# djamahl99/findnpropagate

Measured on AMD Instinct MI355X. Metric: NuScenes scenes/s (30k pts, Transfusion voxel backbone), higher is better.
Workload: dtype bf16

## Files before the change

### findnpropagate_amd/backbones_3d/spconv_backbone.py

```python
from functools import partial

import os
import torch
import torch.nn as nn

from .. import sparse as S
from .. import spconv


def replace_feature(out, new_features):
    return out.replace_feature(new_features)


def post_act_block(in_channels, out_channels, kernel_size, indice_key=None, stride=1, padding=0,
                   conv_type='subm', norm_fn=None):
    if conv_type == 'subm':
        conv = spconv.SubMConv3d(in_channels, out_channels, kernel_size, bias=False, indice_key=indice_key)
    elif conv_type == 'spconv':
        conv = spconv.SparseConv3d(in_channels, out_channels, kernel_size, stride=stride, padding=padding,
                                   bias=False, indice_key=indice_key)
    elif conv_type == 'inverseconv':
        conv = spconv.SparseInverseConv3d(in_channels, out_channels, kernel_size, indice_key=indice_key, bias=False)
    else:
        raise NotImplementedError
# ... 266 lines not shown


TWO_STREAMS = {"0": False, "1": True}.get(os.environ.get("FNP_TWO_STREAMS", ""))


class _PointsGraph:
    FAR = 1.0e9

    def __init__(self, engine, capacity, n_feat, batch_size, voxel_cfg, device, probe=False, split_index=False):
        self.probe, self.deferred = bool(probe), []
        self.host_counts = not self.probe
        self.split_index, self.graph_i, self._index_cut = bool(split_index), None, False
        self.counts_dev = None
        if self.host_counts:
            self.counts_pin = torch.zeros((32,), dtype=torch.int32, pin_memory=True)
            self._pin_np = self.counts_pin.numpy()
            self.counts_seq, self._replays = torch.zeros((1,), dtype=torch.int32, device=device), 0
        else:
            self.counts_pin = torch.empty((16,), dtype=torch.int32, pin_memory=True)
            self.graph_b, self.counts_event = torch.cuda.CUDAGraph(), torch.cuda.Event()
        self.done_event = torch.cuda.Event()
        self._replayed = False
        self.engine, self.capacity, self.batch_size = engine, capacity, batch_size
        self.pts = torch.full((capacity, n_feat), self.FAR, dtype=torch.float32, device=device)
        self.off = torch.zeros((batch_size + 1,), dtype=torch.int32, device=device)
        self.n_prev = 0
        self.prep_key = engine._prep_key
        engine._gate_hold = True
        try:
            self._body(voxel_cfg)
        finally:
            engine._gate_hold = False
        torch.cuda.synchronize(device)
        self.cap_factor = engine._graph_key()
        self.graph = torch.cuda.CUDAGraph()
        import gc
        gc_was_on = gc.isenabled()
        gc.collect()
        gc.disable()
        try:
            if self.split_index:
                self.graph_i = torch.cuda.CUDAGraph()
                self._ctx = torch.cuda.graph(self.graph_i)
            else:
                self._ctx = torch.cuda.graph(self.graph)
            self._ctx.__enter__()
            try:
                self.vox, self.res = self._body(voxel_cfg, capture=True)
            finally:
                self._ctx.__exit__(None, None, None)
            assert self.counts_dev is not None and (self.deferred or not self.probe), "the engine did not reach its cut"
            assert self._index_cut or not self.split_index, "the engine did not cut behind its index chain"
        finally:
            if gc_was_on:
                gc.enable()

    def stage(self, points, batch_offsets):
        n = int(points.shape[0])
        if (points.is_cuda and points.dtype == torch.float32 and points.is_contiguous() and batch_offsets.is_cuda
                and batch_offsets.dtype == torch.int32 and batch_offsets.is_contiguous()):
            S.stage_points(points, batch_offsets, self.pts, self.off, self.n_prev, self.FAR)
        else:
            self.pts[:n].copy_(points, non_blocking=True)
            if self.n_prev > n:
                self.pts[n:self.n_prev].fill_(self.FAR)
            self.off.copy_(batch_offsets, non_blocking=True)
        self.n_prev = n

    def index_ready(self):
        if not self.split_index or self._index_cut:
            return
        self._index_cut = True
        self._ctx.__exit__(None, None, None)
        self._ctx = torch.cuda.graph(self.graph, pool=self.graph_i.pool())
        self._ctx.__enter__()

    def counts_ready(self, counts_dev):
        self.counts_dev = counts_dev
        if self.host_counts:
            return
        self._ctx.__exit__(None, None, None)
        self._ctx = torch.cuda.graph(self.graph_b, pool=(self.graph_i if self.split_index else self.graph).pool())
        self._ctx.__enter__()

    def replay(self, profile=None, conv_stream=None):
        cur = torch.cuda.current_stream(self.pts.device)
        if self._replayed:
            cur.wait_event(self.done_event)
        if self.engine._last_done is not None and self.engine._last_done is not self.done_event:
            cur.wait_event(self.engine._last_done)
# ... 33 lines not shown
        if self.host_counts:
            import time
            want, word, t0 = self._replays & 0xffffffff, self._pin_np, None
            spins = 0
            while (int(word[16]) & 0xffffffff) != want:
                spins += 1
                if spins > 3000:
                    time.sleep(5.0e-5)
                    if spins & 0x3f == 0:
                        t0 = t0 or time.monotonic()
                        if self.done_event.query() and (int(word[16]) & 0xffffffff) != want:
                            raise RuntimeError("the forward ended without its counts launch (sequence %d, expected %d)" % (int(word[16]), want))
                        if time.monotonic() - t0 > 60.0:
                            raise RuntimeError("no counts from the device after 60 s")
            return [int(v) for v in word[:self.counts_dev.numel()]]
        self.counts_event.synchronize()
        return self.counts_pin[:self.counts_dev.numel()].tolist()

    def _body(self, voxel_cfg, capture=False):
        e = self.engine
        e._ensure_clean()
        e._dirty = True
        grids = e._get_grids(self.batch_size, self.pts.device)
        vox = S.voxelize(self.pts, self.off, self.batch_size, voxel_cfg, grid=grids[0], workspace=e._vox_ws)
        e._vox_ws = vox['workspace']
        res = e._run_once(vox['mean'], vox['coords'], vox['n'], self.batch_size, grids[0], sync=False, n_cells=vox['n_cells'],
                          probe=self if capture else None)
        return vox, res


concurrent_streams = S.concurrent_streams


class PointsPipeline:

    def __init__(self, module, batch_size, voxel_cfg, depth=2, capacity=65536, n_feat=5, device=None, probe=False, serial_convs=None, streams=None):
        assert depth >= 1
        self.probe, self.profile = bool(probe), None
        self.module, self.batch_size, self.cfg, self.depth = module, int(batch_size), voxel_cfg, int(depth)
        self.capacity, self.n_feat = int(capacity), int(n_feat)
        self.device = device if device is not None else next(module.parameters()).device
        self.engines = [FusedResBackbone(module) for _ in range(self.depth)]
        for e in self.engines:
            e.two_streams = self.depth == 1

        self.serial_convs = self.depth > 1 and (bool(serial_convs) if serial_convs is not None else self.batch_size >= 8)
        if streams is not None:
# ... 590 lines not shown
```

### findnpropagate_amd/csrc/voxelize.hip

```cpp
#include "rankgrid.h"

namespace {

constexpr int kThreads = 256;
constexpr int kSentinel = 0x7f7f7f7f;
constexpr int kMaxBatch = 1024;

struct VoxWs {
    long long *code;
    int *rank;
    int *flag;
    int *top;
    int *cnt;
    int *scene;
    int *n_sorted;
    int *n_first;
    int *fscan;
    void *scan_ws;
};

__host__ long long align_up(long long v) { return (v + 255) & ~255ll; }

__host__ long long carve(VoxWs &w, char *base, long long n, int B, int cap, int maxp, long long nsum) {
    long long off = 0;
    auto take = [&](long long bytes) {
        char *p = base ? base + off : nullptr;
        off += align_up(bytes);
        return p;
    };
    w.code = (long long *)take(8 * n);
    w.rank = (int *)take(4 * n);
    w.flag = (int *)take(4 * n);
    w.fscan = (int *)take(4 * n);
    w.top = (int *)take(4ll * cap * maxp);
    w.cnt = (int *)take(4ll * cap + 4);
    w.scene = (int *)take(4ll * (3 * B + 8));
    w.n_sorted = (int *)take(4);
    w.n_first = (int *)take(4);
    const long long a = fnp_scan::rank_grid_workspace_bytes(nsum), b2 = fnp_scan::workspace_bytes(n);
    w.scan_ws = take(a > b2 ? a : b2);
    return off;
}

__device__ __forceinline__ int batch_of(const int *__restrict__ off, int B, int i) {
    int lo = 0, hi = B;
    while (hi - lo > 1) {
        const int mid = (lo + hi) >> 1;
        if (off[mid] <= i) lo = mid; else hi = mid;
    }
    return lo;
}

__global__ __launch_bounds__(kThreads) void vox_mark_kernel(const float *__restrict__ pts, int n, int C,
                                                            const int *__restrict__ boff, int B, fnp_voxel_cfg cfg,
                                                            RG g, long long *__restrict__ code, int *__restrict__ cnt) {
    {
        const int z = blockIdx.x * kThreads + threadIdx.x;
        if (z <= n) cnt[z] = 0;
        if (z == 0 && (long long)gridDim.x * kThreads <= n) cnt[n] = 0;
    }
    __shared__ MarkTab tab;
    mark_tab_init(&tab, threadIdx.x, kThreads);
    const int i = blockIdx.x * kThreads + threadIdx.x;
    const int lane = fnp_lane();
    long long blk = -1;
    unsigned long long m = 0ull;
    if (i < n) {
        const float *p = pts + (size_t)i * C;
        int c[3];
        bool ok = true;
#pragma unroll
        for (int j = 0; j < 3; ++j) {
            const float q = (p[j] - cfg.range_min[j]) / cfg.voxel_size[j];
            const float f = floorf(q);
            ok = ok && (f >= 0.f) && (f < (float)cfg.grid[j]);
            c[j] = (int)f;
        }
        long long cd = -1;
        if (ok) {
            const int i0 = __builtin_amdgcn_readfirstlane(i);
            int b = batch_of(boff, B, i0);
            if (b + 1 < B && i >= boff[b + 1]) b = batch_of(boff, B, i);
            blk = rg_block_of(g.d, b, c[2], c[1], c[0]);
            const int bit = rg_bit_of(c[2], c[1], c[0]);
            m = 1ull << bit;
            cd = (blk << 6) | bit;
        }
        code[i] = cd;
    }
#pragma unroll
    for (int d = 1; d < 64; d <<= 1) {
        const long long nb = __shfl_up(blk, d);
        const unsigned long long nm = __shfl_up(m, d);
        if (lane >= d && nb == blk) m |= nm;
    }
    const long long nxt = __shfl_down(blk, 1);
    if (blk >= 0 && (lane == 63 || nxt != blk)) mark_put(&tab, g, blk, m);
    mark_tab_flush(&tab, g, threadIdx.x, kThreads);
}

__global__ __launch_bounds__(kThreads) void vox_insert_kernel(int n, int maxp, int cap,
                                                              const unsigned long long *__restrict__ bits,
                                                              const unsigned *__restrict__ base,
                                                              const long long *__restrict__ code,
                                                              int *__restrict__ rank, int *__restrict__ top, int *__restrict__ cnt,
                                                              int *__restrict__ crowded, int *__restrict__ late) {
    const int i = blockIdx.x * kThreads + threadIdx.x;
    if (i >= n) return;
    late[i] = 0;
    const long long cd = code[i];
    int r = -1;
    if (cd >= 0) {
        const long long blk = cd >> 6;
        const int bit = (int)(cd & 63);
        r = (int)base[blk] + __popcll(bits[blk] & ((1ull << bit) - 1ull));
        if (r >= cap) r = -1;
    }
    rank[i] = r;
    if (r < 0) return;
    const int s = atomicAdd(&cnt[r], 1);
    if (s < maxp) {
// ... 12 lines not shown
    int carry = i;
    int *slots = top + (size_t)rank[i] * maxp;
    for (int j = 0; j < maxp; ++j) {
        const int old = atomicMin(&slots[j], carry);
        carry = old > carry ? old : carry;
    }
}

__global__ __launch_bounds__(kThreads) void vox_flag_kernel(int n, int maxp, const int *__restrict__ rank,
                                                            const int *__restrict__ top, const int *__restrict__ cnt, int *__restrict__ flag) {
    const int i = fnp_xcd_block() * kThreads + threadIdx.x;
    if (i >= n) return;
    const int r = rank[i];
    int f = 0;
    if (r >= 0) {
        const int np = min(cnt[r], maxp);
        int m = kSentinel;
        for (int j = 0; j < np; ++j) m = min(m, top[(size_t)r * maxp + j]);
        f = m == i ? 1 : 0;
    }
    flag[i] = f;
}

__global__ __launch_bounds__(64) void vox_scene_kernel(const int *__restrict__ boff, int B, int n, const int *__restrict__ fc,
                                                       const int *__restrict__ n_first, int max_voxels, int cap,
                                                       int *__restrict__ scene, int *__restrict__ n_voxels) {
    int *fc_start = scene;
    int *out_base = scene + (B + 1);
    const int lane = threadIdx.x;
    const int total = *n_first;
    int acc = 0;
    for (int b0 = 0; b0 < B; b0 += 64) {
        const int b = b0 + lane;
        int c = 0;
        if (b < B) {
            const int o0 = boff[b], o1 = boff[b + 1];
            const int f0 = (o0 < n) ? fc[o0] : total, f1 = (o1 < n) ? fc[o1] : total;
            fc_start[b] = f0;
            if (b == B - 1) fc_start[B] = f1;
            c = min(f1 - f0, max_voxels);
        }
        int inc = c;
#pragma unroll
        for (int d = 1; d < 64; d <<= 1) {
            const int t = __shfl_up(inc, d);
            if (lane >= d) inc += t;
        }
        if (b < B) out_base[b] = acc + inc - c;
        acc += __shfl(inc, 63);
// ... 3 lines not shown
        scene[2 * (B + 1)] = 0;
        *n_voxels = acc;
    }
}

struct CellPts {
    const int *slots;
    int np, s0, s1;
    __device__ __forceinline__ int next_above(int prev) const {
        if (np <= 2) {
            const int a = s0, b = np == 2 ? s1 : kSentinel;
            const int lo = a < b ? a : b, hi = a < b ? b : a;
            return lo > prev ? lo : hi;
        }
        int m = kSentinel;
        for (int j = 0; j < np; ++j) {
            const int v = slots[j];
            m = (v > prev && v < m) ? v : m;
        }
        return m;
    }
};

__device__ __forceinline__ void vox_write_row(const float *__restrict__ pts, int C, int maxp, const CellPts &cp, int p0, int r, int id,
                                              int bb, int z, int y, int x, int *__restrict__ perm, int *__restrict__ coords,
                                              int *__restrict__ num_points, float *__restrict__ mean, float *__restrict__ voxels) {
    const int np = cp.np;
    auto next_above = [&](int prev) -> int { return cp.next_above(prev); };
    perm[r] = id;
    reinterpret_cast<int4 *>(coords)[id] = make_int4(bb, z, y, x);
    num_points[id] = np;
    const float norm = (float)(np < 1 ? 1 : np);
    if ((C == 5 || C == 4) && maxp < 16) {
        typedef float f4u __attribute__((ext_vector_type(4), aligned(4)));
        f4u s4 = {0.f, 0.f, 0.f, 0.f};
        float part[4] = {0.f, 0.f, 0.f, 0.f}, tl[3] = {0.f, 0.f, 0.f};
        const int P4 = maxp & ~3;
        int pi = p0;
        for (int j = 0; j < np; ++j) {
            const float *pr = pts + (size_t)pi * C;
            const f4u v4 = *reinterpret_cast<const f4u *>(pr);
            const float v1 = C == 5 ? pr[4] : 0.f;
            if (j + 1 < np) pi = next_above(pi);
            s4 += v4;
#pragma unroll
            for (int k = 0; k < 4; ++k) part[k] += (j < P4 && (j & 3) == k) ? v1 : 0.f;
#pragma unroll
            for (int k = 0; k < 3; ++k) tl[k] = (j == P4 + k) ? v1 : tl[k];
        }
        float *mo = mean + (size_t)id * C;
        f4u m4 = {s4[0] / norm, s4[1] / norm, s4[2] / norm, s4[3] / norm};
        *reinterpret_cast<f4u *>(mo) = m4;
        if (C == 5) {
            float s1f = part[0];
#pragma unroll
            for (int k = 0; k < 3; ++k) s1f += (P4 + k < maxp) ? tl[k] : 0.f;
            s1f += part[1];
            s1f += part[2];
            s1f += part[3];
            mo[4] = s1f / norm;
        }
    } else {
        for (int c = 0; c < C; ++c) {
            const bool ilp = C < 8 && c >= (C / 4) * 4;
// ... 50 lines not shown
                for (int k = 1; k < 4; ++k) {
#pragma unroll
                    for (int l = 1; l < 4; ++l) acc[k][0] += acc[k][l];
                    sacc += acc[k][0];
                }
            } else {
#pragma unroll
                for (int l = 1; l < 4; ++l) acc[0][0] += acc[0][l];
                sacc = acc[0][0];
            }
            mean[(size_t)id * C + c] = sacc / norm;
        }
    }
    if (voxels) {
        float *v = voxels + (size_t)id * maxp * C;
        int pi = p0;
        for (int j = 0; j < maxp; ++j) {
            for (int c = 0; c < C; ++c) v[j * C + c] = j < np ? pts[(size_t)pi * C + c] : 0.f;
            if (j + 1 < np) pi = next_above(pi);
        }
    }
}

__global__ __launch_bounds__(kThreads) void vox_emit_points_kernel(const float *__restrict__ pts, int n, int C, int maxp,
                                                                   const int *__restrict__ boff, int B, int max_voxels,
                                                                   RankGridDims g, const long long *__restrict__ code,
                                                                   const int *__restrict__ rank, const int *__restrict__ top,
                                                                   const int *__restrict__ cnt, const int *__restrict__ fc,
                                                                   const int *__restrict__ n_first, const int *__restrict__ scene,
                                                                   const int *__restrict__ n_sorted, int cap,
                                                                   int *__restrict__ perm, int *__restrict__ coords,
                                                                   int *__restrict__ num_points, float *__restrict__ mean,
                                                                   float *__restrict__ voxels, int *__restrict__ n_cells,
                                                                   int *__restrict__ n_dropped) {
    const int ns = min(*n_sorted, cap);
    const int *fc_start = scene;
    const int *out_base = scene + (B + 1);
    if (n_cells && blockIdx.x == 0 && threadIdx.x == 0) *n_cells = ns;
    for (int r = ns + blockIdx.x * kThreads + threadIdx.x; r < cap; r += gridDim.x * kThreads) perm[r] = -1;
    const int i = (int)fnp_xcd_block() * kThreads + threadIdx.x;
    if (i >= n) return;
    const int r = rank[i];
    if (r < 0) return;
    const int f0 = fc[i], f1 = i + 1 < n ? fc[i + 1] : *n_first;
    if (f1 == f0) return;
    const long long cd = code[i];
    int bb, z, y, x;
    rg_decode(g, cd >> 6, (int)(cd & 63), bb, z, y, x);
    const int srank = f0 - fc_start[bb];
    const int id = out_base[bb] + srank;
    if (srank >= max_voxels || id >= cap) {
        perm[r] = -1;
        if (n_cells) {
            const int t = out_base[B] + atomicAdd(n_dropped, 1);
            if (t < cap) reinterpret_cast<int4 *>(coords)[t] = make_int4(bb, z, y, x);
        }
        return;
// ... 77 lines not shown
                                                                float *__restrict__ dst, const int *__restrict__ off_src, int n_off,
                                                                int *__restrict__ off_dst) {
    const long long i = (long long)blockIdx.x * kThreads + threadIdx.x;
    if (i < n_words) dst[i] = src[i];
    else if (i < n_prev_words) dst[i] = pad;
    if (i < n_off) off_dst[i] = off_src[i];
}
extern "C" int fnp_stage_points(const float *points, int64_t n_points, int64_t n_prev_points, int num_features, float pad, float *dst_points,
                                const int *batch_offsets, int n_offsets, int *dst_offsets, fnp_stream_t stream) {
    if (n_points < 0 || n_prev_points < 0 || num_features <= 0 || !dst_points || n_offsets < 0 || (n_points > 0 && !points) ||
        (n_offsets > 0 && (!batch_offsets || !dst_offsets)))
        return FNP_ERR_ARG;
    const long long nw = (long long)n_points * num_features, pw = (long long)n_prev_points * num_features;
    const long long span = nw > pw ? nw : pw;
    const long long items = span > n_offsets ? span : n_offsets;
    if (items == 0) return FNP_OK;
    if (items > (long long)kThreads * 0x7fffffff) return FNP_ERR_ARG;
    hipLaunchKernelGGL(stage_points_kernel, dim3((unsigned)((items + kThreads - 1) / kThreads)), dim3(kThreads), 0, (hipStream_t)stream, points, nw, pw, pad,
                       dst_points, batch_offsets, n_offsets, dst_offsets);
    FNP_LAUNCH_CHECK();
    return FNP_OK;
}

extern "C" int fnp_voxelize(const float *points, int n, const int *batch_offsets, const fnp_voxel_cfg *cfg,
                            const fnp_rankgrid *grid, void *workspace, int64_t workspace_bytes, int *coords,
                            int *num_points, float *mean_feats, float *voxels, int *n_voxels, int *n_cells, int cap,
                            fnp_stream_t stream) {
    hipStream_t s = (hipStream_t)stream;
    if (!cfg || n < 0 || cap <= 0 || !n_voxels || !fnp_rg_valid(grid, true) || grid->B > kMaxBatch || !grid_covers(cfg, grid))
        return FNP_ERR_ARG;
    if (cfg->num_features < 3 || cfg->max_points <= 0 || cfg->max_points > 64 || cfg->max_voxels <= 0) return FNP_ERR_ARG;
    if (n == 0) {
        int frc = fnp_fill_words(n_voxels, 1, 0u, s);
        if (!frc && n_cells) frc = fnp_fill_words(n_cells, 1, 0u, s);
        return frc;
    }
    if (!points || !batch_offsets || !workspace || !coords || !num_points || !mean_feats) return FNP_ERR_ARG;
    if (cap < n) return FNP_ERR_ARG;
    const RG g = fnp_rg_view(grid);
    const int B = grid->B;
    VoxWs w;
    const long long need = carve(w, (char *)workspace, n, B, n, cfg->max_points, g.nsum);
    if (need > workspace_bytes) return FNP_ERR_WORKSPACE;
    const int maxp = cfg->max_points, C = cfg->num_features;
    const int pgrid = fnp_divup(n, kThreads);

    hipLaunchKernelGGL(vox_mark_kernel, dim3(pgrid), dim3(kThreads), 0, s, points, n, C, batch_offsets, B, *cfg, g, w.code, w.cnt);
    FNP_LAUNCH_CHECK();
    int rc = fnp_scan::rank_grid(g, w.n_sorted, w.scan_ws, s, nullptr, 0, g.ctr != nullptr);
    if (rc) return rc;
    hipLaunchKernelGGL(vox_insert_kernel, dim3(pgrid), dim3(kThreads), 0, s, n, maxp, n,
                       (const unsigned long long *)g.bits, (const unsigned *)g.base, w.code, w.rank, w.top, w.cnt, w.cnt + n, w.flag);
    FNP_LAUNCH_CHECK();
    hipLaunchKernelGGL(vox_crowded_insert_kernel, dim3(pgrid), dim3(kThreads), 0, s, n, maxp, (const int *)w.rank, (const int *)w.flag, w.top, (const int *)(w.cnt + n));
    FNP_LAUNCH_CHECK();
    hipLaunchKernelGGL(vox_flag_kernel, dim3(pgrid), dim3(kThreads), 0, s, n, maxp, w.rank, w.top, (const int *)w.cnt, w.flag);
    FNP_LAUNCH_CHECK();
    rc = fnp_scan::int32(w.flag, n, w.fscan, w.n_first, w.scan_ws, s);
    if (rc) return rc;
    hipLaunchKernelGGL(vox_scene_kernel, dim3(1), dim3(64), 0, s, batch_offsets, B, n, w.fscan, w.n_first,
                       cfg->max_voxels, cap, w.scene, n_voxels);
    FNP_LAUNCH_CHECK();
    hipLaunchKernelGGL(vox_emit_points_kernel, dim3(pgrid), dim3(kThreads), 0, s, points, n, C, maxp, batch_offsets, B, cfg->max_voxels,
                       g.d, w.code, (const int *)w.rank, w.top, (const int *)w.cnt, w.fscan, (const int *)w.n_first, w.scene, w.n_sorted, n,
                       g.perm, coords, num_points, mean_feats, voxels, n_cells, w.scene + 2 * (B + 1));
    FNP_LAUNCH_CHECK();
    return FNP_OK;
}

extern "C" int fnp_rankgrid_build(const int *coords, const int *n_rows, int cap, const fnp_rankgrid *grid,
                                  void *workspace, int64_t workspace_bytes, fnp_stream_t stream) {
    hipStream_t s = (hipStream_t)stream;
    if (!coords || !n_rows || cap <= 0 || !fnp_rg_valid(grid) || !workspace) return FNP_ERR_ARG;
    const RG g = fnp_rg_view(grid);
    if (fnp_scan::rank_grid_workspace_bytes(g.nsum) + 256 > workspace_bytes) return FNP_ERR_WORKSPACE;
    int *total = (int *)workspace;
    void *scan_ws = (char *)workspace + 256;
    const int blocks = fnp_grid_for(cap, kThreads);
    hipLaunchKernelGGL(rg_mark_coords_kernel<false>, dim3(blocks), dim3(kThreads), 0, s, coords, n_rows, cap, g);
    FNP_LAUNCH_CHECK();
    int rc = fnp_scan::rank_grid(g, total, scan_ws, s);
    if (rc) return rc;
    if (g.perm) {
        {
            const int frc = fnp_fill_words(g.perm, cap, 0xffffffffu, s);
            if (frc) return frc;
        }
        hipLaunchKernelGGL(rg_perm_kernel, dim3(blocks), dim3(kThreads), 0, s, coords, n_rows, cap, g);
        FNP_LAUNCH_CHECK();
    }
// ... 142 lines not shown
```

### findnpropagate_amd/lib.py

```python
import ctypes
import os
import re
from ctypes import POINTER, c_char_p, c_double, c_float, c_int, c_int64, c_uint, c_uint64, c_void_p

_HERE = os.path.dirname(os.path.abspath(__file__))
LIB_PATH = os.environ.get("FNP_LIB_PATH") or os.path.join(_HERE, "libfnp_hip.so")
HEADER_PATH = os.path.join(os.path.dirname(_HERE), "include", "fnp.h")

FNP_F32 = 0
FNP_BF16 = 1
FNP_F16 = 2

FNP_SHUFFLE_NONE = 0
FNP_SHUFFLE_DEVICE = 1
FNP_SHUFFLE_EXPLICIT = 2
FNP_PREP_MAX_STEPS = 6
FNP_SWEEP_DROP_EGO = 1
FNP_SWEEP_TRANSFORM = 2
FNP_SWEEP_FINISHED = 4

_ERRORS = {-1: "FNP_ERR_ARG", -2: "FNP_ERR_LAUNCH", -3: "FNP_ERR_HIP", -4: "FNP_ERR_WORKSPACE"}


class FnpError(RuntimeError):
# ... 63 lines not shown
    "fnp_recall_counters": (c_int, [P, c_int, c_int, P, P, c_int, c_int, P, c_int, c_int, P, c_int, c_uint, c_uint, P, P]),
    "fnp_seeker_pack_records": (c_int, [P, P, P, c_int, P, c_int, c_int, P, P]),
    "fnp_host_points_in_boxes_frame": (c_int, [P, c_int, c_int, P, c_int, P, P]),
    "fnp_host_points_in_boxes_compact": (c_int, [P, c_int64, c_int, P, c_int, P, c_int, c_int64, c_int64, P, c_int64, P, P]),
    "fnp_host_boxes_iou_bev": (c_int, [P, c_int, P, c_int, P]),
    "fnp_host_boxes_aligned_iou_bev": (c_int, [P, P, c_int, P]),
    "fnp_nms_workspace_bytes": (c_int64, [c_int]),
    "fnp_nms_rotated": (c_int, [P, c_int, c_float, P, P, P, P]),
    "fnp_nms_normal": (c_int, [P, c_int, c_float, P, P, P, P]),
    "fnp_nms_batched_workspace_bytes": (c_int64, [c_int, c_int]),
    "fnp_nms_batched": (c_int, [P, P, c_int, c_int, c_float, c_int, P, P, P, P]),
    "fnp_rankgrid_num_blocks": (c_int64, [c_int, c_int, c_int, c_int]),
    "fnp_rankgrid_num_summary": (c_int64, [c_int, c_int, c_int, c_int]),
    "fnp_rankgrid_counter_words": (c_int64, [c_int, c_int, c_int, c_int]),
    "fnp_rankgrid_workspace_bytes": (c_int64, [c_int, c_int, c_int, c_int]),
    "fnp_rankgrid_build": (c_int, [P, P, c_int, POINTER(RankGridC), P, c_int64, P]),
    "fnp_rankgrid_clear": (c_int, [P, P, c_int, POINTER(RankGridC), P]),
    "fnp_rankgrid_clear_multi": (c_int, [c_int, P, P, P, P, P]),
    "fnp_rankgrid_clear_summary": (c_int, [c_int, c_void_p, c_void_p]),
    "fnp_voxelize_workspace_bytes": (c_int64, [c_int64, POINTER(VoxelCfg), POINTER(RankGridC)]),
    "fnp_stage_points": (c_int, [P, c_int64, c_int64, c_int, c_float, P, P, c_int, P, P]),
    "fnp_voxelize": (c_int, [P, c_int, P, POINTER(VoxelCfg), POINTER(RankGridC), P, c_int64,
                             P, P, P, P, P, P, c_int, P]),
    "fnp_host_voxelize": (c_int, [P, c_int, POINTER(VoxelCfg), P, P, P, c_int]),
    "fnp_prepare_points_workspace_bytes": (c_int64, [c_int64]),
    "fnp_prepare_points": (c_int, [P, c_int64, c_int, P, c_int, P, c_int, c_double, c_double, c_double, c_double,
                                   c_int, P, c_int64, c_uint64, c_float, P, c_int64, P, P, P]),
    "fnp_host_cut_records": (c_int, [P, c_int, P]),
    "fnp_host_points_outside_boxes": (c_int, [P, c_int64, c_int, P, c_int, P]),
    "fnp_prepare_points_cut": (c_int, [P, c_int64, c_int, P, c_int, P, c_int, P, P, P, c_double, c_double, c_double, c_double,
                                       c_int, P, c_int64, c_uint64, c_float, P, c_int64, P, P, P]),
    "fnp_prepare_points_cut_window": (c_int, [P, c_int64, c_int, P, c_int, P, c_int, P, P, P, P, c_double, c_double, c_double,
                                              c_double, c_int, P, c_int64, c_uint64, c_float, P, c_int64, P, P, P]),
    "fnp_assemble_sweeps_workspace_bytes": (c_int64, [c_int64]),
    "fnp_assemble_sweeps": (c_int, [P, c_int64, P, c_int, P, c_int, P, P, P, c_double, c_float, P, c_int64, P, P, P]),
    "fnp_assemble_sweeps_window": (c_int, [P, c_int64, P, c_int, P, c_int, P, P, P, c_double, c_float, P, c_int64, P, P, P, P, P]),
    "fnp_rows_in_boxes_workspace_bytes": (c_int64, [c_int64, c_int]),
    "fnp_rows_in_boxes": (c_int, [P, c_int64, c_int, P, c_int, P, c_int, P, P, c_int, P, P, P, c_int64, P, c_int64, P, P, P, P, P]),
    "fnp_rulebook_subm": (c_int, [P, P, c_int, POINTER(ConvGeom), POINTER(RankGridC), P, P]),
    "fnp_rulebook_strided": (c_int, [P, P, c_int, POINTER(ConvGeom), POINTER(RankGridC), POINTER(RankGridC),
                                     P, P, c_int, P, P, c_int64, P]),
    "fnp_spconv_forward": (c_int, [P, c_int, c_int, P, P, c_int, c_int, P, c_int, P, c_int,
                                   P, P, P, c_int, c_int, c_int, c_int, P]),
    "fnp_spconv_forward_strided": (c_int, [P, c_int, c_int, P, POINTER(RankGridC), POINTER(ConvGeom), P, P, c_int, P, c_int,
                                           P, P, c_int, c_int, c_int, P]),
    "fnp_spconv_tiled_aborts": (c_int, []),
# ... 185 lines not shown
```

### findnpropagate_amd/sparse.py

```python
import ctypes
import os
from dataclasses import dataclass
from typing import List, Optional

import torch

from . import lib as _l


def _triple(v):
    if isinstance(v, (list, tuple)):
        assert len(v) == 3
        return [int(x) for x in v]
    return [int(v)] * 3


@dataclass
class RankGrid:
    bits: torch.Tensor
    base: torch.Tensor
    summary: torch.Tensor
    perm: Optional[torch.Tensor]
    batch_size: int
    shape: List[int]
# ... 266 lines not shown
        out = dict(counts=torch.empty((T,), dtype=torch.int32, device=dev), total=torch.empty((1,), dtype=torch.int32, device=dev),
                   indices=torch.empty((capacity,), dtype=torch.int32, device=dev),
                   rows=torch.empty((capacity, 5), dtype=torch.float32, device=dev), capacity=capacity,
                   workspace=torch.empty((ws_bytes,), dtype=torch.uint8, device=dev))
    else:
        assert out["counts"].numel() == T and out["capacity"] == capacity and out["workspace"].numel() >= ws_bytes
    rc = L.fnp_rows_in_boxes(_l.ptr(points) if n else None, n, 5, _l.ptr(batch_offsets), batch_size, _l.ptr(records) if T else None, T,
                             _l.ptr(box_offsets), *cut_args, capacity, _l.ptr(out["workspace"]), out["workspace"].numel(),
                             _l.ptr(out["counts"]) if T else None, _l.ptr(out["total"]), _l.ptr(out["indices"]) if capacity else None,
                             _l.ptr(out["rows"]) if capacity else None, _l.stream())
    _l.check(rc, "fnp_rows_in_boxes")
    return out


def rows_in_boxes_exact(points, batch_offsets, batch_size, records, box_offsets, cut=None, capacity=4096):
    res = rows_in_boxes(points, batch_offsets, batch_size, records, box_offsets, cut=cut, capacity=capacity)
    head = torch.cat([res["total"], res["counts"]]).cpu().numpy()
    total = int(head[0])
    if total > res["capacity"]:
        res = rows_in_boxes(points, batch_offsets, batch_size, records, box_offsets, cut=cut, capacity=total)
    return head[1:].astype("int64"), res["indices"][:total].cpu().numpy(), res["rows"][:total].cpu().numpy()


def voxelize(points, batch_offsets, batch_size, cfg, grid=None, want_voxels=False, workspace=None):
    L = _l.load()
    _l.require_device(points, batch_offsets)
    assert points.dtype == torch.float32 and points.dim() == 2 and points.is_contiguous()
    assert batch_offsets.dtype == torch.int32 and batch_offsets.numel() == batch_size + 1
    n, C = points.shape
    assert C == cfg.num_features
    dev = points.device
    cap = max(n, 1)
    if grid is None:
        grid = alloc_grid(batch_size, [cfg.grid[2], cfg.grid[1], cfg.grid[0]], dev, with_perm_cap=cap)
    elif grid.perm is None or grid.perm.numel() < cap:
        grid.perm = torch.empty((cap,), dtype=torch.int32, device=dev)
    assert grid.batch_size == batch_size
    gc = grid.c()
    ws_bytes = int(L.fnp_voxelize_workspace_bytes(n, cfg, gc))
    _l.check(min(ws_bytes, 0), "fnp_voxelize_workspace_bytes")
    if workspace is None or workspace.numel() < ws_bytes:
        workspace = torch.empty((ws_bytes,), dtype=torch.uint8, device=dev)
    coords = torch.empty((cap, 4), dtype=torch.int32, device=dev)
    num_points = torch.empty((cap,), dtype=torch.int32, device=dev)
    mean = torch.empty((cap, C), dtype=torch.float32, device=dev)
    voxels = torch.empty((cap, cfg.max_points, C), dtype=torch.float32, device=dev) if want_voxels else None
    n_vox = torch.empty((2,), dtype=torch.int32, device=dev)
    rc = L.fnp_voxelize(_l.ptr(points), n, _l.ptr(batch_offsets), cfg, gc,
                        _l.ptr(workspace), workspace.numel(),
                        _l.ptr(coords), _l.ptr(num_points), _l.ptr(mean), _l.ptr(voxels), _l.ptr(n_vox),
                        n_vox.data_ptr() + 4, cap, _l.stream())
    _l.check(rc, "fnp_voxelize")
    return dict(coords=coords, num_points=num_points, mean=mean, voxels=voxels, n=n_vox[:1], n_cells=n_vox[1:],
                grid=grid, workspace=workspace, cap=cap)


def build_grid(indices, n_dev, batch_size, shape, keep_order=True, grid=None):
    L = _l.load()
    _l.require_device(indices, n_dev)
    assert indices.dtype == torch.int32 and indices.is_contiguous()
    cap = max(indices.shape[0], 1)
    dev = indices.device
    if grid is None:
        grid = alloc_grid(batch_size, shape, dev, with_perm_cap=cap if keep_order else None)
    assert grid.batch_size == batch_size and list(grid.shape) == [int(v) for v in shape]
    if keep_order and (grid.perm is None or grid.perm.numel() < cap):
        grid.perm = torch.empty((cap,), dtype=torch.int32, device=dev)
    ws = torch.empty((int(L.fnp_rankgrid_workspace_bytes(batch_size, *grid.shape)) + 256,), dtype=torch.uint8, device=dev)
    rc = L.fnp_rankgrid_build(_l.ptr(indices), _l.ptr(n_dev), cap, grid.c(with_perm=keep_order), _l.ptr(ws), ws.numel(),
                              _l.stream())
    _l.check(rc, "fnp_rankgrid_build")
    return grid


def clear_grid(grid, indices, n_dev):
    L = _l.load()
    rc = L.fnp_rankgrid_clear(_l.ptr(indices), _l.ptr(n_dev), max(indices.shape[0], 1), grid.c(), _l.stream())
# ... 565 lines not shown
```

### include/fnp.h

```cpp
#ifndef FNP_H
#define FNP_H

#include <stdint.h>

#ifdef __cplusplus
extern "C" {
#endif

typedef void *fnp_stream_t;

enum {
    FNP_OK = 0,
    FNP_ERR_ARG = -1,
    FNP_ERR_LAUNCH = -2,
    FNP_ERR_HIP = -3,
    FNP_ERR_WORKSPACE = -4
};

enum { FNP_F32 = 0, FNP_BF16 = 1, FNP_F16 = 2 };

const char *fnp_version(void);
int fnp_abi_version(void);


// ... 67 lines not shown
                             const fnp_rankgrid *grids, fnp_stream_t stream);

int fnp_rankgrid_clear_summary(int count, const fnp_rankgrid *grids, fnp_stream_t stream);

typedef struct fnp_voxel_cfg {
    float range_min[3];
    float voxel_size[3];
    int grid[3];
    int num_features;
    int max_points;
    int max_voxels;
} fnp_voxel_cfg;

int64_t fnp_voxelize_workspace_bytes(int64_t n_points, const fnp_voxel_cfg *cfg, const fnp_rankgrid *grid);

int fnp_stage_points(const float *points, int64_t n_points, int64_t n_prev_points, int num_features, float pad, float *dst_points,
                     const int *batch_offsets, int n_offsets, int *dst_offsets, fnp_stream_t stream);

int fnp_voxelize(const float *points, int n_points, const int *batch_offsets,
                 const fnp_voxel_cfg *cfg, const fnp_rankgrid *grid,
                 void *workspace, int64_t workspace_bytes,
                 int *coords, int *num_points, float *mean_feats, float *voxels,
                 int *n_voxels, int *n_cells, int cap, fnp_stream_t stream);

int fnp_host_voxelize(const float *points, int n_points, const fnp_voxel_cfg *cfg, float *voxels, int *coords,
                      int *num_points, int max_rows);

enum { FNP_SHUFFLE_NONE = 0, FNP_SHUFFLE_DEVICE = 1, FNP_SHUFFLE_EXPLICIT = 2 };
enum { FNP_PREP_MAX_STEPS = 6 };

int64_t fnp_prepare_points_workspace_bytes(int64_t n_points);

int fnp_prepare_points(const float *points, int64_t n_points, int num_features, const int *batch_offsets, int batch_size,
                       const float *program, int program_steps, double x_min, double y_min, double x_max, double y_max,
                       int shuffle_mode, const int *perm, int64_t n_perm, uint64_t seed, float pad,
                       void *workspace, int64_t workspace_bytes, float *out_points, int *out_offsets, fnp_stream_t stream);

int fnp_host_cut_records(const float *boxes, int m, float *records);
int fnp_host_points_outside_boxes(const float *points, int64_t n, int num_features, const float *records, int m,
                                  unsigned char *keep);

int fnp_prepare_points_cut(const float *points, int64_t n_points, int num_features, const int *batch_offsets, int batch_size,
                           const float *program, int program_steps, const float *cut_records, const int *cut_offsets,
                           const int *cut_from, double x_min, double y_min, double x_max, double y_max,
                           int shuffle_mode, const int *perm, int64_t n_perm, uint64_t seed, float pad,
                           void *workspace, int64_t workspace_bytes, float *out_points, int *out_offsets, fnp_stream_t stream);
// ... 302 lines not shown
```

Measured before the change: 13740.

## Read frame points through a device pointer cell instead of staging copies

Instead of copying each frame's points into a fixed FAR-padded staging buffer before graph replay, the captured graph now reads a small device-side cell that holds the current points pointer, offsets pointer and point count. A tiny kernel updates the cell per frame, and the voxelize kernels dereference it and mask work beyond the real count. This removes the staging copy and pad fill for device-resident inputs. In exchange it adds an extra wait on the previous replay's done event, one more launch per frame, and indirect loads inside the kernels.

```diff
diff --git a/findnpropagate_amd/backbones_3d/spconv_backbone.py b/findnpropagate_amd/backbones_3d/spconv_backbone.py
--- a/findnpropagate_amd/backbones_3d/spconv_backbone.py
+++ b/findnpropagate_amd/backbones_3d/spconv_backbone.py
@@ -312,9 +312,12 @@
         self.done_event = torch.cuda.Event()
         self._replayed = False
         self.engine, self.capacity, self.batch_size = engine, capacity, batch_size
-        self.pts = torch.full((capacity, n_feat), self.FAR, dtype=torch.float32, device=device)
+        self.pts = torch.empty((capacity, n_feat), dtype=torch.float32, device=device)
         self.off = torch.zeros((batch_size + 1,), dtype=torch.int32, device=device)
-        self.n_prev = 0
+        self.n_feat = int(n_feat)
+        self.cell = S.frame_cell_alloc(device)
+        S.frame_cell_set(self.cell, self.pts[:0], self.off)
+        self.frame = None
         self.prep_key = engine._prep_key
         engine._gate_hold = True
         try:
@@ -347,15 +350,17 @@
 
     def stage(self, points, batch_offsets):
         n = int(points.shape[0])
-        if (points.is_cuda and points.dtype == torch.float32 and points.is_contiguous() and batch_offsets.is_cuda
+        assert n <= self.capacity and batch_offsets.numel() == self.batch_size + 1
+        cur = torch.cuda.current_stream(self.pts.device)
+        if self._replayed:
+            cur.wait_event(self.done_event)
+        if not (points.is_cuda and points.dtype == torch.float32 and points.is_contiguous() and batch_offsets.is_cuda
                 and batch_offsets.dtype == torch.int32 and batch_offsets.is_contiguous()):
-            S.stage_points(points, batch_offsets, self.pts, self.off, self.n_prev, self.FAR)
-        else:
             self.pts[:n].copy_(points, non_blocking=True)
-            if self.n_prev > n:
-                self.pts[n:self.n_prev].fill_(self.FAR)
             self.off.copy_(batch_offsets, non_blocking=True)
-        self.n_prev = n
+            points, batch_offsets = self.pts[:n], self.off
+        S.frame_cell_set(self.cell, points, batch_offsets)
+        self.frame = (points, batch_offsets)
 
     def index_ready(self):
         if not self.split_index or self._index_cut:
@@ -435,7 +440,7 @@
         e._ensure_clean()
         e._dirty = True
         grids = e._get_grids(self.batch_size, self.pts.device)
-        vox = S.voxelize(self.pts, self.off, self.batch_size, voxel_cfg, grid=grids[0], workspace=e._vox_ws)
+        vox = S.voxelize_cell(self.cell, self.capacity, self.n_feat, self.batch_size, voxel_cfg, grid=grids[0], workspace=e._vox_ws)
         e._vox_ws = vox['workspace']
         res = e._run_once(vox['mean'], vox['coords'], vox['n'], self.batch_size, grids[0], sync=False, n_cells=vox['n_cells'],
                           probe=self if capture else None)
diff --git a/findnpropagate_amd/csrc/voxelize.hip b/findnpropagate_amd/csrc/voxelize.hip
--- a/findnpropagate_amd/csrc/voxelize.hip
+++ b/findnpropagate_amd/csrc/voxelize.hip
@@ -42,7 +42,11 @@
     return off;
 }
 
-__device__ __forceinline__ int batch_of(const int *__restrict__ off, int B, int i) {
+#define FNP_GLOBAL __attribute__((address_space(1)))
+typedef const FNP_GLOBAL float *gfloat_p;
+typedef const FNP_GLOBAL int *gint_p;
+
+__device__ __forceinline__ int batch_of(gint_p __restrict__ off, int B, int i) {
     int lo = 0, hi = B;
     while (hi - lo > 1) {
         const int mid = (lo + hi) >> 1;
@@ -51,14 +55,26 @@
     return lo;
 }
 
-__global__ __launch_bounds__(kThreads) void vox_mark_kernel(const float *__restrict__ pts, int n, int C,
-                                                            const int *__restrict__ boff, int B, fnp_voxel_cfg cfg,
+struct Frame {
+    gfloat_p pts;
+    gint_p boff;
+    int n;
+};
+template <bool CELL>
+__device__ __forceinline__ Frame frame_of(const float *pts, const int *boff, int n, const fnp_frame_cell *__restrict__ cell) {
+    if (!CELL) return Frame{(gfloat_p)pts, (gint_p)boff, n};
+    const long long m = cell->n_points;
+    return Frame{(gfloat_p)cell->points, (gint_p)cell->batch_offsets, (int)(m < 0 ? 0 : (m < n ? m : n))};
+}
+
+template <bool CELL>
+__global__ __launch_bounds__(kThreads) void vox_mark_kernel(const float *__restrict__ pts_, int n, int C,
+                                                            const int *__restrict__ boff_, const fnp_frame_cell *__restrict__ cell,
+                                                            int B, fnp_voxel_cfg cfg,
                                                             RG g, long long *__restrict__ code, int *__restrict__ cnt) {
-    {
-        const int z = blockIdx.x * kThreads + threadIdx.x;
-        if (z <= n) cnt[z] = 0;
-        if (z == 0 && (long long)gridDim.x * kThreads <= n) cnt[n] = 0;
-    }
+    const Frame fr = frame_of<CELL>(pts_, boff_, n, cell);
+    const gfloat_p __restrict__ pts = fr.pts;
+    const gint_p __restrict__ boff = fr.boff;
     __shared__ MarkTab tab;
     mark_tab_init(&tab, threadIdx.x, kThreads);
     const int i = blockIdx.x * kThreads + threadIdx.x;
@@ -66,25 +82,27 @@
     long long blk = -1;
     unsigned long long m = 0ull;
     if (i < n) {
-        const float *p = pts + (size_t)i * C;
-        int c[3];
-        bool ok = true;
-#pragma unroll
-        for (int j = 0; j < 3; ++j) {
-            const float q = (p[j] - cfg.range_min[j]) / cfg.voxel_size[j];
-            const float f = floorf(q);
-            ok = ok && (f >= 0.f) && (f < (float)cfg.grid[j]);
-            c[j] = (int)f;
-        }
         long long cd = -1;
-        if (ok) {
-            const int i0 = __builtin_amdgcn_readfirstlane(i);
-            int b = batch_of(boff, B, i0);
-            if (b + 1 < B && i >= boff[b + 1]) b = batch_of(boff, B, i);
-            blk = rg_block_of(g.d, b, c[2], c[1], c[0]);
-            const int bit = rg_bit_of(c[2], c[1], c[0]);
-            m = 1ull << bit;
-            cd = (blk << 6) | bit;
+        if (i < fr.n) {
+            const gfloat_p p = pts + (size_t)i * C;
+            int c[3];
+            bool ok = true;
+#pragma unroll
+            for (int j = 0; j < 3; ++j) {
+                const float q = (p[j] - cfg.range_min[j]) / cfg.voxel_size[j];
+                const float f = floorf(q);
+                ok = ok && (f >= 0.f) && (f < (float)cfg.grid[j]);
+                c[j] = (int)f;
+            }
+            if (ok) {
+                const int i0 = __builtin_amdgcn_readfirstlane(i);
+                int b = batch_of(boff, B, i0);
+                if (b + 1 < B && i >= boff[b + 1]) b = batch_of(boff, B, i);
+                blk = rg_block_of(g.d, b, c[2], c[1], c[0]);
+                const int bit = rg_bit_of(c[2], c[1], c[0]);
+                m = 1ull << bit;
+                cd = (blk << 6) | bit;
+            }
         }
         code[i] = cd;
     }
@@ -97,6 +115,8 @@
     const long long nxt = __shfl_down(blk, 1);
     if (blk >= 0 && (lane == 63 || nxt != blk)) mark_put(&tab, g, blk, m);
     mark_tab_flush(&tab, g, threadIdx.x, kThreads);
+    if (i <= n) cnt[i] = 0;
+    if (i == 0 && (long long)gridDim.x * kThreads <= n) cnt[n] = 0;
 }
 
 __global__ __launch_bounds__(kThreads) void vox_insert_kernel(int n, int maxp, int cap,
@@ -155,9 +175,12 @@
     flag[i] = f;
 }
 
-__global__ __launch_bounds__(64) void vox_scene_kernel(const int *__restrict__ boff, int B, int n, const int *__restrict__ fc,
+template <bool CELL>
+__global__ __launch_bounds__(64) void vox_scene_kernel(const int *__restrict__ boff_, const fnp_frame_cell *__restrict__ cell, int B, int n,
+                                                       const int *__restrict__ fc,
                                                        const int *__restrict__ n_first, int max_voxels, int cap,
                                                        int *__restrict__ scene, int *__restrict__ n_voxels) {
+    const gint_p __restrict__ boff = frame_of<CELL>(nullptr, boff_, n, cell).boff;
     int *fc_start = scene;
     int *out_base = scene + (B + 1);
     const int lane = threadIdx.x;
@@ -207,7 +230,7 @@
     }
 };
 
-__device__ __forceinline__ void vox_write_row(const float *__restrict__ pts, int C, int maxp, const CellPts &cp, int p0, int r, int id,
+__device__ __forceinline__ void vox_write_row(const gfloat_p __restrict__ pts, int C, int maxp, const CellPts &cp, int p0, int r, int id,
                                               int bb, int z, int y, int x, int *__restrict__ perm, int *__restrict__ coords,
                                               int *__restrict__ num_points, float *__restrict__ mean, float *__restrict__ voxels) {
     const int np = cp.np;
@@ -223,8 +246,8 @@
         const int P4 = maxp & ~3;
         int pi = p0;
         for (int j = 0; j < np; ++j) {
-            const float *pr = pts + (size_t)pi * C;
-            const f4u v4 = *reinterpret_cast<const f4u *>(pr);
+            const gfloat_p pr = pts + (size_t)pi * C;
+            const f4u v4 = *(const FNP_GLOBAL f4u *)pr;
             const float v1 = C == 5 ? pr[4] : 0.f;
             if (j + 1 < np) pi = next_above(pi);
             s4 += v4;
@@ -321,8 +344,9 @@
     }
 }
 
-__global__ __launch_bounds__(kThreads) void vox_emit_points_kernel(const float *__restrict__ pts, int n, int C, int maxp,
-                                                                   const int *__restrict__ boff, int B, int max_voxels,
+template <bool CELL>
+__global__ __launch_bounds__(kThreads) void vox_emit_points_kernel(const float *__restrict__ pts_, const fnp_frame_cell *__restrict__ cell,
+                                                                   int n, int C, int maxp, int B, int max_voxels,
                                                                    RankGridDims g, const long long *__restrict__ code,
                                                                    const int *__restrict__ rank, const int *__restrict__ top,
                                                                    const int *__restrict__ cnt, const int *__restrict__ fc,
@@ -332,6 +356,7 @@
                                                                    int *__restrict__ num_points, float *__restrict__ mean,
                                                                    float *__restrict__ voxels, int *__restrict__ n_cells,
                                                                    int *__restrict__ n_dropped) {
+    const gfloat_p __restrict__ pts = frame_of<CELL>(pts_, nullptr, n, cell).pts;
     const int ns = min(*n_sorted, cap);
     const int *fc_start = scene;
     const int *out_base = scene + (B + 1);
@@ -455,20 +480,11 @@
     return FNP_OK;
 }
 
-extern "C" int fnp_voxelize(const float *points, int n, const int *batch_offsets, const fnp_voxel_cfg *cfg,
-                            const fnp_rankgrid *grid, void *workspace, int64_t workspace_bytes, int *coords,
-                            int *num_points, float *mean_feats, float *voxels, int *n_voxels, int *n_cells, int cap,
-                            fnp_stream_t stream) {
-    hipStream_t s = (hipStream_t)stream;
-    if (!cfg || n < 0 || cap <= 0 || !n_voxels || !fnp_rg_valid(grid, true) || grid->B > kMaxBatch || !grid_covers(cfg, grid))
-        return FNP_ERR_ARG;
-    if (cfg->num_features < 3 || cfg->max_points <= 0 || cfg->max_points > 64 || cfg->max_voxels <= 0) return FNP_ERR_ARG;
-    if (n == 0) {
-        int frc = fnp_fill_words(n_voxels, 1, 0u, s);
-        if (!frc && n_cells) frc = fnp_fill_words(n_cells, 1, 0u, s);
-        return frc;
-    }
-    if (!points || !batch_offsets || !workspace || !coords || !num_points || !mean_feats) return FNP_ERR_ARG;
+template <bool CELL>
+static int voxelize_launch(const float *points, const int *batch_offsets, const fnp_frame_cell *cell, int n, const fnp_voxel_cfg *cfg,
+                           const fnp_rankgrid *grid, void *workspace, int64_t workspace_bytes, int *coords, int *num_points,
+                           float *mean_feats, float *voxels, int *n_voxels, int *n_cells, int cap, hipStream_t s) {
+    if (!workspace || !coords || !num_points || !mean_feats) return FNP_ERR_ARG;
     if (cap < n) return FNP_ERR_ARG;
     const RG g = fnp_rg_view(grid);
     const int B = grid->B;
@@ -478,27 +494,73 @@
     const int maxp = cfg->max_points, C = cfg->num_features;
     const int pgrid = fnp_divup(n, kThreads);
 
-    hipLaunchKernelGGL(vox_mark_kernel, dim3(pgrid), dim3(kThreads), 0, s, points, n, C, batch_offsets, B, *cfg, g, w.code, w.cnt);
+    hipLaunchKernelGGL(vox_mark_kernel<CELL>, dim3(pgrid), dim3(kThreads), 0, s, points, n, C, batch_offsets, cell, B, *cfg, g, w.code, w.cnt);
     FNP_LAUNCH_CHECK();
     int rc = fnp_scan::rank_grid(g, w.n_sorted, w.scan_ws, s, nullptr, 0, g.ctr != nullptr);
     if (rc) return rc;
     hipLaunchKernelGGL(vox_insert_kernel, dim3(pgrid), dim3(kThreads), 0, s, n, maxp, n,
                        (const unsigned long long *)g.bits, (const unsigned *)g.base, w.code, w.rank, w.top, w.cnt, w.cnt + n, w.flag);
     FNP_LAUNCH_CHECK();
-    hipLaunchKernelGGL(vox_crowded_insert_kernel, dim3(pgrid), dim3(kThreads), 0, s, n, maxp, (const int *)w.rank, (const int *)w.flag, w.top, (const int *)(w.cnt + n));
+    hipLaunchKernelGGL(vox_crowded_insert_kernel, dim3(pgrid), dim3(kThreads), 0, s, n, maxp,
+                       (const int *)w.rank, (const int *)w.flag, w.top, (const int *)(w.cnt + n));
     FNP_LAUNCH_CHECK();
     hipLaunchKernelGGL(vox_flag_kernel, dim3(pgrid), dim3(kThreads), 0, s, n, maxp, w.rank, w.top, (const int *)w.cnt, w.flag);
     FNP_LAUNCH_CHECK();
     rc = fnp_scan::int32(w.flag, n, w.fscan, w.n_first, w.scan_ws, s);
     if (rc) return rc;
-    hipLaunchKernelGGL(vox_scene_kernel, dim3(1), dim3(64), 0, s, batch_offsets, B, n, w.fscan, w.n_first,
+    hipLaunchKernelGGL(vox_scene_kernel<CELL>, dim3(1), dim3(64), 0, s, batch_offsets, cell, B, n, w.fscan, w.n_first,
                        cfg->max_voxels, cap, w.scene, n_voxels);
     FNP_LAUNCH_CHECK();
-    hipLaunchKernelGGL(vox_emit_points_kernel, dim3(pgrid), dim3(kThreads), 0, s, points, n, C, maxp, batch_offsets, B, cfg->max_voxels,
+    hipLaunchKernelGGL(vox_emit_points_kernel<CELL>, dim3(pgrid), dim3(kThreads), 0, s, points, cell, n, C, maxp, B, cfg->max_voxels,
                        g.d, w.code, (const int *)w.rank, w.top, (const int *)w.cnt, w.fscan, (const int *)w.n_first, w.scene, w.n_sorted, n,
                        g.perm, coords, num_points, mean_feats, voxels, n_cells, w.scene + 2 * (B + 1));
     FNP_LAUNCH_CHECK();
     return FNP_OK;
+}
+
+static bool voxelize_args_ok(const fnp_voxel_cfg *cfg, int n, int cap, const int *n_voxels, const fnp_rankgrid *grid) {
+    if (!cfg || n < 0 || cap <= 0 || !n_voxels || !fnp_rg_valid(grid, true) || grid->B > kMaxBatch || !grid_covers(cfg, grid)) return false;
+    return !(cfg->num_features < 3 || cfg->max_points <= 0 || cfg->max_points > 64 || cfg->max_voxels <= 0);
+}
+
+extern "C" int fnp_voxelize(const float *points, int n, const int *batch_offsets, const fnp_voxel_cfg *cfg,
+                            const fnp_rankgrid *grid, void *workspace, int64_t workspace_bytes, int *coords,
+                            int *num_points, float *mean_feats, float *voxels, int *n_voxels, int *n_cells, int cap,
+                            fnp_stream_t stream) {
+    hipStream_t s = (hipStream_t)stream;
+    if (!voxelize_args_ok(cfg, n, cap, n_voxels, grid)) return FNP_ERR_ARG;
+    if (n == 0) {
+        int frc = fnp_fill_words(n_voxels, 1, 0u, s);
+        if (!frc && n_cells) frc = fnp_fill_words(n_cells, 1, 0u, s);
+        return frc;
+    }
+    if (!points || !batch_offsets) return FNP_ERR_ARG;
+    return voxelize_launch<false>(points, batch_offsets, nullptr, n, cfg, grid, workspace, workspace_bytes, coords, num_points, mean_feats,
+                                  voxels, n_voxels, n_cells, cap, s);
+}
+
+__global__ __launch_bounds__(64) void frame_cell_set_kernel(fnp_frame_cell *__restrict__ cell, const float *points, const int *batch_offsets,
+                                                            long long n_points) {
+    if (threadIdx.x == 0) {
+        cell->points = points;
+        cell->batch_offsets = batch_offsets;
+        cell->n_points = n_points;
+    }
+}
+extern "C" int fnp_frame_cell_set(fnp_frame_cell *cell, const float *points, const int *batch_offsets, int64_t n_points, fnp_stream_t stream) {
+    if (!cell || ((uintptr_t)cell & 7) || n_points < 0 || (n_points > 0 && !points) || !batch_offsets) return FNP_ERR_ARG;
+    hipLaunchKernelGGL(frame_cell_set_kernel, dim3(1), dim3(64), 0, (hipStream_t)stream, cell, points, batch_offsets, (long long)n_points);
+    FNP_LAUNCH_CHECK();
+    return FNP_OK;
+}
+
+extern "C" int fnp_voxelize_cell(const fnp_frame_cell *cell, int max_points_in_frame, const fnp_voxel_cfg *cfg, const fnp_rankgrid *grid,
+                                 void *workspace, int64_t workspace_bytes, int *coords, int *num_points, float *mean_feats, float *voxels,
+                                 int *n_voxels, int *n_cells, int cap, fnp_stream_t stream) {
+    if (!cell || ((uintptr_t)cell & 7) || max_points_in_frame <= 0 || !voxelize_args_ok(cfg, max_points_in_frame, cap, n_voxels, grid))
+        return FNP_ERR_ARG;
+    return voxelize_launch<true>(nullptr, nullptr, cell, max_points_in_frame, cfg, grid, workspace, workspace_bytes, coords, num_points,
+                                 mean_feats, voxels, n_voxels, n_cells, cap, (hipStream_t)stream);
 }
 
 extern "C" int fnp_rankgrid_build(const int *coords, const int *n_rows, int cap, const fnp_rankgrid *grid,
diff --git a/findnpropagate_amd/lib.py b/findnpropagate_amd/lib.py
--- a/findnpropagate_amd/lib.py
+++ b/findnpropagate_amd/lib.py
@@ -109,6 +109,9 @@
     "fnp_stage_points": (c_int, [P, c_int64, c_int64, c_int, c_float, P, P, c_int, P, P]),
     "fnp_voxelize": (c_int, [P, c_int, P, POINTER(VoxelCfg), POINTER(RankGridC), P, c_int64,
                              P, P, P, P, P, P, c_int, P]),
+    "fnp_frame_cell_set": (c_int, [P, P, P, c_int64, P]),
+    "fnp_voxelize_cell": (c_int, [P, c_int, POINTER(VoxelCfg), POINTER(RankGridC), P, c_int64,
+                                  P, P, P, P, P, P, c_int, P]),
     "fnp_host_voxelize": (c_int, [P, c_int, POINTER(VoxelCfg), P, P, P, c_int]),
     "fnp_prepare_points_workspace_bytes": (c_int64, [c_int64]),
     "fnp_prepare_points": (c_int, [P, c_int64, c_int, P, c_int, P, c_int, c_double, c_double, c_double, c_double,
diff --git a/findnpropagate_amd/sparse.py b/findnpropagate_amd/sparse.py
--- a/findnpropagate_amd/sparse.py
+++ b/findnpropagate_amd/sparse.py
@@ -312,14 +312,9 @@
     return head[1:].astype("int64"), res["indices"][:total].cpu().numpy(), res["rows"][:total].cpu().numpy()
 
 
-def voxelize(points, batch_offsets, batch_size, cfg, grid=None, want_voxels=False, workspace=None):
-    L = _l.load()
-    _l.require_device(points, batch_offsets)
-    assert points.dtype == torch.float32 and points.dim() == 2 and points.is_contiguous()
-    assert batch_offsets.dtype == torch.int32 and batch_offsets.numel() == batch_size + 1
-    n, C = points.shape
+def _voxelize_call(entry, name, head, n, C, batch_size, cfg, grid, want_voxels, workspace, dev):
+    L = _l.load()
     assert C == cfg.num_features
-    dev = points.device
     cap = max(n, 1)
     if grid is None:
         grid = alloc_grid(batch_size, [cfg.grid[2], cfg.grid[1], cfg.grid[0]], dev, with_perm_cap=cap)
@@ -336,13 +331,42 @@
     mean = torch.empty((cap, C), dtype=torch.float32, device=dev)
     voxels = torch.empty((cap, cfg.max_points, C), dtype=torch.float32, device=dev) if want_voxels else None
     n_vox = torch.empty((2,), dtype=torch.int32, device=dev)
-    rc = L.fnp_voxelize(_l.ptr(points), n, _l.ptr(batch_offsets), cfg, gc,
-                        _l.ptr(workspace), workspace.numel(),
-                        _l.ptr(coords), _l.ptr(num_points), _l.ptr(mean), _l.ptr(voxels), _l.ptr(n_vox),
-                        n_vox.data_ptr() + 4, cap, _l.stream())
-    _l.check(rc, "fnp_voxelize")
+    rc = entry(*head, cfg, gc, _l.ptr(workspace), workspace.numel(),
+               _l.ptr(coords), _l.ptr(num_points), _l.ptr(mean), _l.ptr(voxels), _l.ptr(n_vox),
+               n_vox.data_ptr() + 4, cap, _l.stream())
+    _l.check(rc, name)
     return dict(coords=coords, num_points=num_points, mean=mean, voxels=voxels, n=n_vox[:1], n_cells=n_vox[1:],
                 grid=grid, workspace=workspace, cap=cap)
+
+
+def voxelize(points, batch_offsets, batch_size, cfg, grid=None, want_voxels=False, workspace=None):
+    _l.require_device(points, batch_offsets)
+    assert points.dtype == torch.float32 and points.dim() == 2 and points.is_contiguous()
+    assert batch_offsets.dtype == torch.int32 and batch_offsets.numel() == batch_size + 1
+    n, C = points.shape
+    return _voxelize_call(_l.load().fnp_voxelize, "fnp_voxelize", (_l.ptr(points), n, _l.ptr(batch_offsets)), n, C, batch_size, cfg,
+                          grid, want_voxels, workspace, points.device)
+
+
+def frame_cell_alloc(device):
+    return torch.zeros((4,), dtype=torch.int64, device=device)
+
+
+def frame_cell_set(cell, points, batch_offsets):
+    _l.require_device(cell, points, batch_offsets)
+    assert cell.dtype == torch.int64 and cell.numel() >= 3 and cell.is_contiguous()
+    assert points.dtype == torch.float32 and points.dim() == 2 and points.is_contiguous()
+    assert batch_offsets.dtype == torch.int32 and batch_offsets.is_contiguous()
+    n = int(points.shape[0])
+    _l.check(_l.load().fnp_frame_cell_set(_l.ptr(cell), _l.ptr(points) if n else None, _l.ptr(batch_offsets), n, _l.stream()), "fnp_frame_cell_set")
+
+
+def voxelize_cell(cell, max_points_in_frame, n_feat, batch_size, cfg, grid=None, want_voxels=False, workspace=None):
+    _l.require_device(cell)
+    n = int(max_points_in_frame)
+    assert n > 0 and cell.dtype == torch.int64 and cell.numel() >= 3
+    return _voxelize_call(_l.load().fnp_voxelize_cell, "fnp_voxelize_cell", (_l.ptr(cell), n), n, int(n_feat), batch_size, cfg,
+                          grid, want_voxels, workspace, cell.device)
 
 
 def build_grid(indices, n_dev, batch_size, shape, keep_order=True, grid=None):
diff --git a/include/fnp.h b/include/fnp.h
--- a/include/fnp.h
+++ b/include/fnp.h
@@ -113,6 +113,19 @@
                  void *workspace, int64_t workspace_bytes,
                  int *coords, int *num_points, float *mean_feats, float *voxels,
                  int *n_voxels, int *n_cells, int cap, fnp_stream_t stream);
+
+typedef struct fnp_frame_cell {
+    const float *points;
+    const int *batch_offsets;
+    int64_t n_points;
+} fnp_frame_cell;
+int fnp_frame_cell_set(fnp_frame_cell *cell, const float *points, const int *batch_offsets, int64_t n_points, fnp_stream_t stream);
+
+int fnp_voxelize_cell(const fnp_frame_cell *cell, int max_points_in_frame,
+                      const fnp_voxel_cfg *cfg, const fnp_rankgrid *grid,
+                      void *workspace, int64_t workspace_bytes,
+                      int *coords, int *num_points, float *mean_feats, float *voxels,
+                      int *n_voxels, int *n_cells, int cap, fnp_stream_t stream);
 
 int fnp_host_voxelize(const float *points, int n_points, const fnp_voxel_cfg *cfg, float *voxels, int *coords,
                       int *num_points, int max_rows);
```

After: 13820 (median of 4 runs). No clear change (+0.5%).
